# stdstu12/YUME

Hardware: AMD Instinct MI355X
Metric: denoise-steps/sec (Yume-5B 720P, 33-frame latent) (higher is better)
Workload: dtype bf16; 1 GPU; Yume-5B-720P random-init, 33-frame 704x1280 clip (latent 48x13x44x80, FramePack lfz=8, L=9460), ODE Euler steps of a 50-step shift-7 schedule, no CFG, one chain per GPU; num_layers=30, parallelism=dp1 (independent chains, replicated weights)

## Files before the change

include/yume_hip.h:

```cpp
#ifndef YUME_HIP_H
#define YUME_HIP_H

#include <stdint.h>

#ifdef __cplusplus
extern "C" {
#endif

#define YUME_OK 0
#define YUME_EINVAL (-1)
#define YUME_ELAUNCH (-2)
#define YUME_EUNSUP (-3)

const char* yume_last_error(void);
#define YUME_ABI_VERSION 9
int yume_abi_version(void);
const char* yume_target_arch(void);

int64_t yume_counter_workspace_bytes(void);
int yume_counter_workspace_init(void* ptr, int64_t bytes, void* stream);

int yume_calibrate_mfma(int64_t iters, int64_t workgroups, void* ticks, void* sink, void* stream);

int yume_adaln_modulate(const float* x, int64_t ldx, int64_t T, int64_t C, float eps,
                        const float* mul, const float* add, int64_t tab_stride,
                        const int32_t* row_idx, int add_one,
                        void* out, int64_t ldo, int out_kind, void* stream);

enum {
    YUME_EPI_BF16 = 0,
    YUME_EPI_BF16_GELU = 1,
    YUME_EPI_F32 = 2,
    YUME_EPI_RESID = 3,
    YUME_EPI_BF16_SPLITT = 4,
    YUME_EPI_BF16_GELU_ERF = 5,
    YUME_EPI_BF16_GEGLU = 6,
    YUME_EPI_MX_GELU = 7
};
int yume_gemm_bf16(const void* A, int64_t lda, const void* W, int64_t ldw, const float* bias,
                   int64_t M, int64_t N, int64_t K, int epi,
                   void* out, int64_t ldo,
                   const float* gate, int64_t gate_stride, const int32_t* row_idx,
                   void* outT, int64_t ldt, int64_t n_split,
                   int variant, void* stream);

int64_t yume_gemm_workspace_bytes(void);
int yume_gemm_bf16_ws(const void* A, int64_t lda, const void* W, int64_t ldw, const float* bias,
                      int64_t M, int64_t N, int64_t K, int epi,
                      void* out, int64_t ldo,
                      const float* gate, int64_t gate_stride, const int32_t* row_idx,
                      void* outT, int64_t ldt, int64_t n_split,
                      int variant, void* workspace, int64_t workspace_bytes, void* stream);

int yume_quant_rows_e4m3(const void* x, int64_t ldx, int64_t R, int64_t K, void* q, int64_t ldq, float* scale, void* stream);
int yume_gemm_f8(const void* Aq, int64_t lda, const float* sa, const void* Wq, int64_t ldw, const float* sw,
                 const float* bias, int64_t M, int64_t N, int64_t K, int epi, void* out, int64_t ldo,
                 const float* gate, int64_t gate_stride, const int32_t* row_idx, void* stream);
int yume_gemm_f8_splitt(const void* Aq, int64_t lda, const float* sa, const void* Wq, int64_t ldw, const float* sw,
                        const float* bias, int64_t M, int64_t N, int64_t K,
                        void* out, int64_t ldo, void* outT, int64_t ldt, int64_t n_split, void* stream);

int yume_adaln_modulate_e4m3(const float* x, int64_t ldx, int64_t T, int64_t C, float eps, const float* mul,
                             const float* add, int64_t tab_stride, const int32_t* row_idx, int add_one,
                             void* q, int64_t ldq, float* scale, void* stream);
int yume_gemm_f8_mxout(const void* Aq, int64_t lda, const float* sa, const void* Wq, int64_t ldw, const float* sw,
                       const float* bias, int64_t M, int64_t N, int64_t K, int epi, void* out, int64_t ldo,
                       void* eo, int64_t ldeo, void* stream);
int yume_gemm_f8_mx(const void* Aq, int64_t lda, const void* ea, int64_t ldea, const void* Wq, int64_t ldw, const float* sw,
                    const float* bias, int64_t M, int64_t N, int64_t K, int epi, void* out, int64_t ldo,
                    const float* gate, int64_t gate_stride, const int32_t* row_idx, void* stream);

int yume_rmsnorm_rope(void* buf, int64_t ld, int64_t T, int64_t C, int nparts,
                      const float* w, float eps, const float* rope, int64_t D, void* stream);
int yume_rmsnorm_rows_periodic(void* buf, int64_t ld, int64_t T, int64_t C, const float* w, int64_t wperiod, float eps,
                               void* stream);

#define YUME_ATTN_Q_PRESCALED 0x100
#define YUME_ATTN_KV_PADDED 0x200
int yume_attn_fwd(const void* Q, int64_t ldq, const void* K, int64_t ldk, const void* Vt, int64_t ldvt,
                  void* O, int64_t ldo, int64_t Lq, int64_t Lk, int64_t H, float scale,
                  int accumulate, int variant, void* stream);
int64_t yume_attn_workspace_bytes(int64_t Lq, int64_t Lk, int64_t H);
int yume_attn_fwd_ws(const void* Q, int64_t ldq, const void* K, int64_t ldk, const void* Vt, int64_t ldvt,
                     void* O, int64_t ldo, int64_t Lq, int64_t Lk, int64_t H, float scale,
                     int accumulate, int variant, void* workspace, int64_t workspace_bytes, void* stream);
int yume_attn_fwd_kw(const void* Q, int64_t ldq, const void* K, int64_t ldk, const void* Vt, int64_t ldvt,
                     void* O, int64_t ldo, int64_t Lq, int64_t Lk, int64_t H, float scale,
                     int accumulate, int variant, void* workspace, int64_t workspace_bytes, float last_key_weight, void* stream);
int yume_attn_fwd_seg(const void* Q, int64_t ldq, const void* const* K, int64_t ldk, const void* const* Vt, int64_t ldvt,
                      void* O, int64_t ldo, int64_t nseg, int64_t Lq_seg, int64_t seg_pitch, const int64_t* Lk, int64_t H,
                      float scale, int accumulate, int variant, const float* last_key_weight, void* stream);
int64_t yume_attn_batch_workspace_bytes(int64_t nseg, int64_t Lq_seg, int64_t Lk_seg, int64_t H);
int yume_attn_fwd_batch(const void* Q, int64_t ldq, const void* K, int64_t ldk, const void* Vt, int64_t ldvt,
                        void* O, int64_t ldo, int64_t nseg, int64_t Lq_seg, int64_t q_pitch,
                        int64_t Lk_seg, int64_t k_pitch, int64_t H, float scale, int accumulate, int variant,
                        void* workspace, int64_t workspace_bytes, void* stream);

int yume_quant_rows_mx_e4m3(const void* x, int64_t ldx, int64_t R, int64_t K, void* q, int64_t ldq, void* e, int64_t lde, void* stream);
int yume_attn_vt_mx_e4m3(const void* Vt, int64_t ldvt, int64_t C, int64_t Lk, void* Vt8, int64_t ldvt8, void* Ev, int64_t ldev, void* stream);
int yume_attn_fwd_f8mx(const void* Q8, int64_t ldq, const void* Eq, int64_t ldeq, const void* K8, int64_t ldk, const void* Ek, int64_t ldek,
                       const void* Vt8, int64_t ldvt8, const void* Ev, int64_t ldev, void* O, int64_t ldo,
                       int64_t Lq, int64_t Lk, int64_t H, void* stream);

int yume_linear_smallm_f32(const float* in, int64_t R, int64_t K, const void* W, int w_bf16,
                           const float* bias, int64_t N, int in_act, int out_act,
                           const float* add_table, float* out, void* stream);

int yume_sinusoidal_embed(const double* t, const int32_t* t_index, int64_t R, int64_t dim,
                          float* out, void* stream);

int yume_modulation_table(const float* tab, const float* e0, int64_t B, int64_t R, int64_t W,
                          float* out, void* stream);

int yume_patch_gather(const void* x, int in_bf16, int64_t Cin, int64_t F, int64_t H, int64_t W,
                      int64_t f0, int64_t nf, int64_t kh, int64_t kw,
                      void* out, int64_t Kp, void* stream);

int yume_unpatchify(const float* in, int64_t ldi, int64_t Fr, int64_t Hp, int64_t Wp,
                    int64_t ph, int64_t pw, int64_t Cout, float* out, void* stream);

int yume_cast_bf16(const float* in, int64_t ldi, int64_t rows_valid, int64_t rows, int64_t cols,
                   void* out, int64_t ldo, void* stream);
int yume_transpose_bf16(const void* in, int in_bf16, int64_t ldi, int64_t rows, int64_t cols,
                        void* out, int64_t ldo, void* stream);


enum { YUME_CONV_EPI_ADD = 16, YUME_CONV_EPI_TSPLIT = 17, YUME_CONV_EPI_RMS_SILU = 18 };
int yume_conv3d_cl(const void* x, const void* cache, int64_t ldc, int64_t Tin, int64_t Hin, int64_t Win, int64_t Cin,
                   const void* W, int64_t ldw, const float* bias, int64_t Cout,
                   int kt, int kh, int kw, int st, int sh, int sw, int pt, int ph, int pw, int ups,
                   int64_t To, int64_t Ho, int64_t Wo, int epi, void* out, int64_t ldo,
                   const void* add, int64_t ldadd, const void* zero_page, void* stream);

int yume_vae_rmsnorm_silu(const void* x, int64_t ldx, int64_t M, int64_t C, const float* gamma, const float* beta,
                          int silu, void* y, int64_t ldy, void* stream);
// ... 45 lines not shown
```

yume_amd/_lib.py:

```python
import ctypes
import os
from ctypes import c_void_p, c_int, c_int64, c_float, c_char_p

_HERE = os.path.dirname(os.path.abspath(__file__))
LIB_PATH = os.environ.get("YUME_HIP_LIB") or os.path.join(_HERE, "lib", "libyume_hip.so")

_P, _I, _L, _F = c_void_p, c_int, c_int64, c_float

SIGNATURES = {
    "yume_last_error": [],
    "yume_abi_version": [],
    "yume_target_arch": [],
    "yume_counter_workspace_bytes": [],
    "yume_counter_workspace_init": [_P, _L, _P],
    "yume_calibrate_mfma": [_L, _L, _P, _P, _P],
    "yume_adaln_modulate": [_P, _L, _L, _L, _F, _P, _P, _L, _P, _I, _P, _L, _I, _P],
    "yume_adaln_modulate_e4m3": [_P, _L, _L, _L, _F, _P, _P, _L, _P, _I, _P, _L, _P, _P],
    "yume_gemm_bf16": [_P, _L, _P, _L, _P, _L, _L, _L, _I, _P, _L, _P, _L, _P, _P, _L, _L, _I, _P],
    "yume_gemm_workspace_bytes": [],
    "yume_gemm_bf16_ws": [_P, _L, _P, _L, _P, _L, _L, _L, _I, _P, _L, _P, _L, _P, _P, _L, _L, _I, _P, _L, _P],
    "yume_quant_rows_e4m3": [_P, _L, _L, _L, _P, _L, _P, _P],
    "yume_gemm_f8": [_P, _L, _P, _P, _L, _P, _P, _L, _L, _L, _I, _P, _L, _P, _L, _P, _P],
    "yume_gemm_f8_splitt": [_P, _L, _P, _P, _L, _P, _P, _L, _L, _L, _P, _L, _P, _L, _L, _P],
    "yume_gemm_f8_mxout": [_P, _L, _P, _P, _L, _P, _P, _L, _L, _L, _I, _P, _L, _P, _L, _P],
    "yume_gemm_f8_mx": [_P, _L, _P, _L, _P, _L, _P, _P, _L, _L, _L, _I, _P, _L, _P, _L, _P, _P],
    "yume_rmsnorm_f32": [_P, _L, _L, _L, _F, _P, _P, _L, _P],
    "yume_gemm_bf16_batched": [_P, _L, _L, _P, _L, _L, _L, _L, _L, _I, _P, _L, _L, _L, _I, _P],
    "yume_gemm_splitk_workspace_bytes": [_L, _L, _I],
    "yume_gemm_bf16_splitk": [_P, _L, _P, _L, _P, _L, _L, _L, _I, _P, _L, _I, _P, _P],
    "yume_softmax_bias_rows": [_P, _L, _L, _L, _L, _P, _L, _P, _L, _L, _P],
    "yume_rmsnorm_rows_periodic": [_P, _L, _L, _L, _P, _L, _F, _P],
    "yume_rmsnorm_rope": [_P, _L, _L, _L, _I, _P, _F, _P, _L, _P],
    "yume_attn_fwd": [_P, _L, _P, _L, _P, _L, _P, _L, _L, _L, _L, _F, _I, _I, _P],
    "yume_attn_workspace_bytes": [_L, _L, _L],
    "yume_attn_fwd_ws": [_P, _L, _P, _L, _P, _L, _P, _L, _L, _L, _L, _F, _I, _I, _P, _L, _P],
    "yume_attn_fwd_kw": [_P, _L, _P, _L, _P, _L, _P, _L, _L, _L, _L, _F, _I, _I, _P, _L, _F, _P],
    "yume_attn_fwd_seg": [_P, _L, _P, _L, _P, _L, _P, _L, _L, _L, _L, _P, _L, _F, _I, _I, _P, _P],
    "yume_attn_batch_workspace_bytes": [_L, _L, _L, _L],
    "yume_attn_fwd_batch": [_P, _L, _P, _L, _P, _L, _P, _L, _L, _L, _L, _L, _L, _L, _F, _I, _I, _P, _L, _P],
    "yume_quant_rows_mx_e4m3": [_P, _L, _L, _L, _P, _L, _P, _L, _P],
    "yume_attn_vt_mx_e4m3": [_P, _L, _L, _L, _P, _L, _P, _L, _P],
    "yume_attn_fwd_f8mx": [_P, _L, _P, _L, _P, _L, _P, _L, _P, _L, _P, _L, _P, _L, _L, _L, _L, _P],
    "yume_linear_smallm_f32": [_P, _L, _L, _P, _I, _P, _L, _I, _I, _P, _P, _P],
    "yume_sinusoidal_embed": [_P, _P, _L, _L, _P, _P],
    "yume_modulation_table": [_P, _P, _L, _L, _L, _P, _P],
    "yume_patch_gather": [_P, _I, _L, _L, _L, _L, _L, _L, _L, _L, _P, _L, _P],
    "yume_unpatchify": [_P, _L, _L, _L, _L, _L, _L, _L, _P, _P],
    "yume_cast_bf16": [_P, _L, _L, _L, _L, _P, _L, _P],
    "yume_transpose_bf16": [_P, _I, _L, _L, _L, _P, _L, _P],
    "yume_conv3d_cl": [_P, _P, _L, _L, _L, _L, _L, _P, _L, _P, _L, _I, _I, _I, _I, _I, _I, _I, _I, _I, _I, _L, _L, _L, _I, _P, _L,
                       _P, _L, _P, _P],
    "yume_vae_rmsnorm_silu": [_P, _L, _L, _L, _P, _P, _I, _P, _L, _P],
    "yume_vae_rmsnorm_silu_mx": [_P, _L, _L, _L, _P, _P, _I, _P, _L, _P, _L, _P],
    "yume_conv3d_cl_f8mx": [_P, _P, _P, _P, _L, _L, _L, _L, _L, _L, _P, _L, _P, _P, _L, _I, _I, _I, _I, _I, _I, _I, _I, _I, _I, _L, _L, _L,
                            _I, _P, _L, _P, _L, _P, _P],
    "yume_conv_up2_fold": [_P, _L, _L, _L, _L, _L, _P, _L, _P, _L, _P, _L, _P],
    "yume_vae_dupup_add": [_P, _L, _L, _L, _L, _L, _P, _L, _L, _L, _I, _I, _I, _P],
    "yume_vae_avgdown_add": [_P, _L, _L, _L, _L, _L, _P, _L, _L, _I, _I, _P],
    "yume_softmax_rows": [_P, _L, _L, _L, _F, _P, _L, _P],
    "yume_vae_pack_input": [_P, _I, _L, _L, _L, _L, _I, _P, _P, _P, _L, _P],
    "yume_frames_u8": [_P, _L, _L, _L, _L, _P, _P],
    "yume_frames_u8_trunc": [_P, _L, _L, _L, _L, _P, _P],
    "yume_vae_unpack_output": [_P, _L, _L, _L, _L, _L, _I, _P, _P, _F, _F, _P, _P],
}
_RES = {"yume_last_error": c_char_p, "yume_target_arch": c_char_p, "yume_gemm_splitk_workspace_bytes": c_int64, "yume_attn_workspace_bytes": c_int64,
        "yume_attn_batch_workspace_bytes": c_int64,
        "yume_counter_workspace_bytes": c_int64, "yume_gemm_workspace_bytes": c_int64}

_lib = None
ABI_VERSION = 9


def load():
    global _lib
    if _lib is not None:
        return _lib
    if not os.path.exists(LIB_PATH):
        raise RuntimeError(
            f"{LIB_PATH} is missing: the HIP extension has not been built. "
            "Run `python -c 'import __graft_entry__ as g; g.build()'` (or `python -m yume_amd.build`). "
            "There is no CPU/PyTorch fallback for the yume_amd hot path.")
    import torch
    lib = ctypes.CDLL(LIB_PATH)
    for name, argtypes in SIGNATURES.items():
        fn = getattr(lib, name)
        fn.argtypes = argtypes
        fn.restype = _RES.get(name, c_int)
    got, arch = int(lib.yume_abi_version()), lib.yume_target_arch()
    if got != ABI_VERSION or arch != b"gfx950":
        raise RuntimeError(f"{LIB_PATH} has ABI version {got} for {arch!r}, this binding needs {ABI_VERSION} for gfx950: "
                           "rebuild with `python -m yume_amd.build --force`")
    _lib = lib
    return lib


def check(rc, what):
    if rc != 0:
        msg = load().yume_last_error()
        raise RuntimeError(f"{what} failed (rc={rc}): {msg.decode() if msg else '?'}")
```

yume_amd/csrc/gemm_bf16.hip:

```cpp
#include "gemm_core.hpp"
#include "gemm_w4.hpp"

using namespace gemm_core;

namespace {
bool w4_auto() {
    static const bool on = [] { const char* v = getenv("YUME_GEMM_W4"); return !v || atoi(v) != 0; }();
    return on;
}
bool gemm_log() {
    static const bool on = [] { const char* v = getenv("YUME_GEMM_LOG"); return v && atoi(v) != 0; }();
    return on;
}
void gemm_log_line(const char* kernel, int64_t M, int64_t N, int64_t K, int epi, int variant, int64_t lda, int64_t ldw, int64_t ldo, int64_t ldt,
                   int64_t n_split, bool ws, int64_t batch) {
    fprintf(stderr, "[gemm_bf16] %s M=%lld N=%lld K=%lld epi=%d variant=%d lda=%lld ldw=%lld ldo=%lld ldt=%lld n_split=%lld ws=%d batch=%lld\n", kernel,
            (long long)M, (long long)N, (long long)K, epi, variant, (long long)lda, (long long)ldw, (long long)ldo, (long long)ldt, (long long)n_split,
            ws ? 1 : 0, (long long)batch);
}
}

extern "C" int64_t yume_gemm_workspace_bytes(void) { return gemm_w4::sk_workspace_bytes(gemm_w4::SK_MAX_SLOTS); }

extern "C" int yume_gemm_bf16(const void* A, int64_t lda, const void* W, int64_t ldw, const float* bias, int64_t M,
                              int64_t N, int64_t K, int epi, void* out, int64_t ldo, const float* gate,
                              int64_t gate_stride, const int32_t* row_idx, void* outT, int64_t ldt, int64_t n_split,
                              int variant, void* stream) {
    return yume_gemm_bf16_ws(A, lda, W, ldw, bias, M, N, K, epi, out, ldo, gate, gate_stride, row_idx, outT, ldt, n_split, variant, nullptr, 0, stream);
}

extern "C" int yume_gemm_bf16_ws(const void* A, int64_t lda, const void* W, int64_t ldw, const float* bias, int64_t M,
                                 int64_t N, int64_t K, int epi, void* out, int64_t ldo, const float* gate,
                                 int64_t gate_stride, const int32_t* row_idx, void* outT, int64_t ldt, int64_t n_split,
                                 int variant, void* workspace, int64_t workspace_bytes, void* stream) {
    YUME_REQUIRE(A && W && out, "gemm_bf16: NULL pointer");
    YUME_REQUIRE(M > 0 && N > 0 && K > 0, "gemm_bf16: empty problem M=%lld N=%lld K=%lld", (long long)M, (long long)N, (long long)K);
    YUME_REQUIRE(M < (1ll << 31) && N < (1ll << 31) && K < (1ll << 31), "gemm_bf16: dimension too large");
    YUME_REQUIRE((K % BK) == 0, "gemm_bf16: K=%lld must be a multiple of %d", (long long)K, BK);
    YUME_REQUIRE((N % 4) == 0, "gemm_bf16: N=%lld must be a multiple of 4", (long long)N);
    YUME_REQUIRE((lda % 8) == 0 && (ldw % 8) == 0, "gemm_bf16: lda/ldw must be multiples of 8 (16-byte rows)");
    YUME_REQUIRE((ldo % 4) == 0, "gemm_bf16: ldo must be a multiple of 4");
    YUME_REQUIRE(((uintptr_t)A % 16) == 0 && ((uintptr_t)W % 16) == 0 && ((uintptr_t)out % 16) == 0, "gemm_bf16: pointers must be 16-byte aligned");
    Problem p;
    p.W = (const unsigned short*)W; p.ldw = ldw;
    p.M = (int)M; p.N = (int)N; p.K = (int)K;
    p.tiles_m = (int)((M + BM - 1) / BM);
    p.tiles_n = (int)((N + BN - 1) / BN);
    p.group_m = 8;
    p.bsW = 0; p.bsO = 0;
    bool sk = false;
    if (variant == 0 && workspace != nullptr && w4_auto() && epi != YUME_EPI_BF16_GEGLU &&
        use_256(p, 0, epi != YUME_EPI_BF16_SPLITT || (n_split % 256) == 0) && gemm_w4::w4_applies(p, lda, epi) &&
        (epi != YUME_EPI_BF16_SPLITT || (ldt % 8) == 0)) {
        Problem q = p;
        q.tiles_m = (int)((M + 255) / 256);
        q.tiles_n = (int)((N + 255) / 256);
        gemm_w4::w4_sk_plan(q, workspace, workspace_bytes);
        sk = q.sk_wgs != 0;
    }
    if (!sk && variant == 0 && epi != YUME_EPI_BF16_GEGLU && use_256(p, 0, epi != YUME_EPI_BF16_SPLITT || (n_split % 256) == 0)) {
        const int64_t tn = (N + 255) / 256, tm = (M + 255) / 256, T = tm * tn, R = T % 256, full = T - R;
        const int64_t m_main = full / tn, M_main = m_main * 256, rem = M - M_main;
        if (R > 0 && R <= 96 && full >= 256 && m_main >= 1 && rem > 0 && rem <= 1024) {
            const int64_t osz = (epi == YUME_EPI_F32 || epi == YUME_EPI_RESID) ? 4 : 2;
            auto remainder = [&](void* s2) {
                return yume_gemm_bf16(reinterpret_cast<const unsigned short*>(A) + M_main * lda, lda, W, ldw, bias, rem, N, K, epi,
                                      reinterpret_cast<char*>(out) + M_main * ldo * osz, ldo, gate, gate_stride,
                                      row_idx ? row_idx + M_main : nullptr,
                                      outT ? reinterpret_cast<unsigned short*>(outT) + M_main : nullptr, ldt, n_split, 1, s2);
            };
            int rc = yume_gemm_bf16(A, lda, W, ldw, bias, M_main, N, K, epi, out, ldo, gate, gate_stride, row_idx, outT, ldt, n_split,
                                    w4_auto() ? 3 : 2, stream);
            if (rc != YUME_OK) return rc;
            return remainder(stream);
        }
    }
    PlainA al;
    al.A = (const unsigned short*)A; al.lda = lda; al.M = (int)M; al.bsA = 0;
    Epilogue e = {};
    e.bias = bias;
    e.out = out; e.ldo = ldo;
    e.gate = gate; e.gate_stride = gate_stride; e.row_idx = row_idx;
    e.outT = (unsigned short*)outT; e.ldt = ldt; e.n_split = (int)n_split;
    hipStream_t st = (hipStream_t)stream;
    const bool split_ok = epi != YUME_EPI_BF16_SPLITT || (n_split % 256) == 0;
    const bool big = use_256(p, variant == 3 ? 2 : variant, split_ok);
    const bool w4 = (variant == 3 || (variant == 0 && big && w4_auto())) && split_ok && gemm_w4::w4_applies(p, lda, epi) &&
                    (epi != YUME_EPI_BF16_SPLITT || (ldt % 8) == 0);
    if (gemm_log())
        gemm_log_line(epi == YUME_EPI_BF16_GEGLU ? "g256" : w4 ? (sk ? "w4+sk" : "w4") : big ? "g256" : "g128", M, N, K, epi, variant, lda, ldw, ldo, ldt,
                      n_split, workspace != nullptr, 1);
#define YUME_GO(E) (w4 ? gemm_w4::launch_w4(E, p, al, e, st, "gemm_bf16", variant == 0 ? workspace : nullptr, workspace_bytes) : big ? launch256<E>(p, al, e, st, "gemm_bf16") : launch<E>(p, al, e, st, "gemm_bf16"))
    switch (epi) {
        case YUME_EPI_BF16: return YUME_GO(YUME_EPI_BF16);
        case YUME_EPI_BF16_GELU: return YUME_GO(YUME_EPI_BF16_GELU);
        case YUME_EPI_BF16_GELU_ERF: return YUME_GO(YUME_EPI_BF16_GELU_ERF);
        case YUME_EPI_F32: return YUME_GO(YUME_EPI_F32);
        case YUME_EPI_RESID:
            YUME_REQUIRE(gate == nullptr || (gate_stride % 4) == 0, "gemm_bf16: gate_stride must be a multiple of 4");
            return YUME_GO(YUME_EPI_RESID);
        case YUME_EPI_BF16_GEGLU:
            YUME_REQUIRE((N % 8) == 0 && bias == nullptr, "gemm_bf16: GEGLU needs N %% 8 == 0 and no bias");
            return launch256<YUME_EPI_BF16_GEGLU>(p, al, e, st, "gemm_bf16");
        case YUME_EPI_BF16_SPLITT:
            YUME_REQUIRE(outT != nullptr && n_split >= 0 && (n_split % BN) == 0 && ldt >= M && (ldt % 4) == 0,
                         "gemm_bf16: SPLITT needs outT, n_split %% 128 == 0, ldt >= M and ldt %% 4 == 0");
            YUME_REQUIRE(((uintptr_t)outT % 16) == 0, "gemm_bf16: outT must be 16-byte aligned");
            return YUME_GO(YUME_EPI_BF16_SPLITT);
        default:
            yume_set_error("gemm_bf16: unknown epilogue %d", epi);
            return YUME_EINVAL;
    }
}

extern "C" int yume_gemm_bf16_batched(const void* A, int64_t lda, int64_t strideA, const void* W, int64_t ldw, int64_t strideW,
                                      int64_t M, int64_t N, int64_t K, int epi, void* out, int64_t ldo, int64_t strideO,
                                      int64_t batch, int variant, void* stream) {
    (void)variant;
    YUME_REQUIRE(A && W && out, "gemm_bf16_batched: NULL pointer");
    YUME_REQUIRE(epi == YUME_EPI_BF16 || epi == YUME_EPI_F32, "gemm_bf16_batched: only the plain bf16 / fp32 epilogues");
    YUME_REQUIRE(batch >= 1 && batch <= 65535, "gemm_bf16_batched: batch %lld", (long long)batch);
    YUME_REQUIRE(M > 0 && N > 0 && K > 0 && M < (1ll << 31) && N < (1ll << 31) && K < (1ll << 31), "gemm_bf16_batched: bad problem size");
    YUME_REQUIRE((K % BK) == 0 && (N % 4) == 0, "gemm_bf16_batched: K must be a multiple of %d and N of 4", BK);
    YUME_REQUIRE((lda % 8) == 0 && (ldw % 8) == 0 && (ldo % 4) == 0, "gemm_bf16_batched: lda/ldw must be multiples of 8, ldo of 4");
    YUME_REQUIRE((strideA % 8) == 0 && (strideW % 8) == 0 && (strideO % 8) == 0, "gemm_bf16_batched: strides must keep 16-byte alignment");
    YUME_REQUIRE(((uintptr_t)A % 16) == 0 && ((uintptr_t)W % 16) == 0 && ((uintptr_t)out % 16) == 0, "gemm_bf16_batched: pointers must be 16-byte aligned");
    Problem p;
    p.W = (const unsigned short*)W; p.ldw = ldw;
    p.M = (int)M; p.N = (int)N; p.K = (int)K;
    p.tiles_m = (int)((M + BM - 1) / BM);
    p.tiles_n = (int)((N + BN - 1) / BN);
    p.group_m = 8;
    p.bsW = strideW;
    p.bsO = strideO * (epi == YUME_EPI_F32 ? 4 : 2);
    PlainA al;
    al.A = (const unsigned short*)A; al.lda = lda; al.M = (int)M; al.bsA = strideA;
    Epilogue e = {};
    e.out = out; e.ldo = ldo;
    hipStream_t st = (hipStream_t)stream;
    if (gemm_log()) gemm_log_line("batched", M, N, K, epi, variant, lda, ldw, ldo, 0, 0, false, batch);
    if (epi == YUME_EPI_F32) return launch<YUME_EPI_F32>(p, al, e, st, "gemm_bf16_batched", (int)batch);
    return launch<YUME_EPI_BF16>(p, al, e, st, "gemm_bf16_batched", (int)batch);
}

namespace {
template <int EPI>
__global__ __launch_bounds__(256) void splitk_reduce_kernel(const float* __restrict__ ws, int splits, int64_t MN, int N,
                                                            const float* __restrict__ bias, void* __restrict__ out, int64_t ldo) {
    const int64_t nq = MN >> 2;
    for (int64_t i = (int64_t)blockIdx.x * blockDim.x + threadIdx.x; i < nq; i += (int64_t)gridDim.x * blockDim.x) {
        f32x4 v = *reinterpret_cast<const f32x4*>(ws + 4 * i);
        for (int s = 1; s < splits; ++s) v += *reinterpret_cast<const f32x4*>(ws + s * MN + 4 * i);
        const int64_t m = (4 * i) / N;
        const int n = (int)((4 * i) - m * N);
        if (bias) v += *reinterpret_cast<const f32x4*>(bias + n);
        if (EPI == YUME_EPI_F32) {
            *reinterpret_cast<f32x4*>(reinterpret_cast<float*>(out) + m * ldo + n) = v;
        } else if (EPI == YUME_EPI_RESID) {
            float* xo = reinterpret_cast<float*>(out) + m * ldo + n;
            *reinterpret_cast<f32x4*>(xo) = *reinterpret_cast<const f32x4*>(xo) + v;
        } else if (EPI == YUME_EPI_BF16_GEGLU) {
            const unsigned o = pack_bf16x2(v[1] * gelu_tanh(v[0]), v[3] * gelu_tanh(v[2]));
            *reinterpret_cast<unsigned*>(reinterpret_cast<unsigned short*>(out) + m * ldo + (n >> 1)) = o;
        } else {
            if (EPI == YUME_EPI_BF16_GELU) {
#pragma unroll
                for (int q = 0; q < 4; ++q) v[q] = gelu_tanh(v[q]);
// ... 50 lines not shown
```

yume_amd/csrc/gemm_w4.hpp:

```cpp
#pragma once
#include "gemm_core.hpp"
#include "trace.hpp"

namespace gemm_w4 {
using namespace gemm_core;

constexpr int NTHR_W4 = 256;
constexpr int OPER_BYTES = 256 * 128;
constexpr int BUF_BYTES = 2 * OPER_BYTES;
constexpr int LDS_W4 = 2 * BUF_BYTES;

#define W4_AG8(n) "a" #n "0", "a" #n "1", "a" #n "2", "a" #n "3", "a" #n "4", "a" #n "5", "a" #n "6", "a" #n "7", "a" #n "8", "a" #n "9"
#define W4_AGPRS "a0", "a1", "a2", "a3", "a4", "a5", "a6", "a7", "a8", "a9", W4_AG8(1), W4_AG8(2), W4_AG8(3), W4_AG8(4), W4_AG8(5), W4_AG8(6), \
    W4_AG8(7), W4_AG8(8), W4_AG8(9), W4_AG8(10), W4_AG8(11), W4_AG8(12), W4_AG8(13), W4_AG8(14), W4_AG8(15), W4_AG8(16), W4_AG8(17), W4_AG8(18), \
    W4_AG8(19), W4_AG8(20), W4_AG8(21), W4_AG8(22), W4_AG8(23), W4_AG8(24), "a250", "a251", "a252", "a253", "a254", "a255"

#define W4_MFMA2(T0, X0, Y0, T1, X1, Y1)                                                                                                         \
    asm volatile("v_mfma_f32_16x16x32_bf16 a[%c4:%c5], %0, %1, a[%c4:%c5]\n\tv_mfma_f32_16x16x32_bf16 a[%c6:%c7], %2, %3, a[%c6:%c7]"             \
                 ::"v"(X0), "v"(Y0), "v"(X1), "v"(Y1), "n"((T0) * 4), "n"((T0) * 4 + 3), "n"((T1) * 4), "n"((T1) * 4 + 3) : "memory", W4_AGPRS)
#define W4_MFMA2_DMA(T0, X0, Y0, T1, X1, Y1, voff, sbase, lbase, loff)                                                                            \
    asm volatile("s_add_u32 m0, %10, %11\n\tv_mfma_f32_16x16x32_bf16 a[%c4:%c5], %0, %1, a[%c4:%c5]\n\tglobal_load_lds_dwordx4 %8, %9\n\t"         \
                 "v_mfma_f32_16x16x32_bf16 a[%c6:%c7], %2, %3, a[%c6:%c7]"                                                                       \
                 ::"v"(X0), "v"(Y0), "v"(X1), "v"(Y1), "n"((T0) * 4), "n"((T0) * 4 + 3), "n"((T1) * 4), "n"((T1) * 4 + 3), "v"(voff), "s"(sbase),   \
                 "s"(lbase), "n"(loff) : "memory", "scc", W4_AGPRS)
// ... 550 lines not shown
            tails = true;
            const int ntail = (p.sk_s - 1) * R;
            pc0 = (w - R) * p.sk_q;
            pc1 = min(ntail, pc0 + p.sk_q);
            if (pc0 >= pc1) return;
        }
    }
    for (int pc = pc0; pc < pc1; ++pc) {
        int t = head_t, j = 0, k0 = 0, k1 = nk, slot = -1, nslice = 1;
        if (p.sk_wgs && (int)blockIdx.x >= ndp) {
            if (tails) {
                j = 1 + pc / R;
                t = pc - (j - 1) * R;
                k0 = p.sk_lh + (j - 1) * p.sk_lt;
                k1 = j == p.sk_s - 1 ? nk : k0 + p.sk_lt;
                slot = pc;
            } else {
                k1 = p.sk_lh;
                nslice = p.sk_s;
            }
        }
        int m0, n0;
        tile_origin(p, tile0 + t, m0, n0);
        if (epi == YUME_EPI_BF16_SPLITT && n0 >= e.n_split) {
            w4_mainloop<false>(p, al, smem, m0, n0, k0, k1 - k0);
            w4_finish_piece<false>(p, e, epi, smem, m0, n0, slot, t, nslice);
        } else {
            w4_mainloop<true>(p, al, smem, m0, n0, k0, k1 - k0);
            w4_finish_piece<true>(p, e, epi, smem, m0, n0, slot, t, nslice);
        }
        if (pc + 1 < pc1) __syncthreads();
    }
    TRACE_STAMP(2);
}

inline bool w4_applies(const Problem& p, int64_t lda, int epi) {
    if (p.K < 3 * BK) return false;
#ifdef W4_EXPERIMENT
    if (epi != YUME_EPI_BF16) return false;
#endif
    if (255ll * lda * 2 + 128 >= (1ll << 32) || 255ll * p.ldw * 2 + 128 >= (1ll << 32)) return false;
    return epi == YUME_EPI_BF16 || epi == YUME_EPI_BF16_GELU || epi == YUME_EPI_BF16_GELU_ERF || epi == YUME_EPI_F32 || epi == YUME_EPI_RESID ||
           epi == YUME_EPI_BF16_SPLITT;
}

inline void w4_sk_plan(Problem& p, void* ws, int64_t ws_bytes) {
    p.sk_dp = 0; p.sk_tiles = 0; p.sk_wgs = 0; p.sk_s = 1; p.sk_q = 1; p.sk_lh = 0; p.sk_lt = 0; p.sk_ws = nullptr;
    static const bool on = [] { const char* v = getenv("YUME_GEMM_SK"); return !v || atoi(v) != 0; }();
    static const int ncu = [] {
        int d = 0, n = 0;
        if (hipGetDevice(&d) != hipSuccess || hipDeviceGetAttribute(&n, hipDeviceAttributeMultiprocessorCount, d) != hipSuccess) n = 0;
        return n;
    }();
    if (!on || ws == nullptr || ncu < 64 || ncu > SK_MAX_SLOTS || (ncu & 7) != 0) return;
    if (ws_bytes < sk_workspace_bytes(SK_MAX_SLOTS) || ((uintptr_t)ws & 15) != 0) return;
    const int T = p.tiles_m * p.tiles_n, nk = p.K / BK;
    const int R = T % ncu;
    if (R == 0 || T < ncu) return;
    static const int min_nk = [] { const char* v = getenv("YUME_GEMM_SK_MIN_NK"); return v ? atoi(v) : 96; }();
    if (nk < min_nk) return;
    int s, q, lh, lt;
    if (2 * R > ncu) {
        s = 2;
        q = (R + (ncu - R) - 1) / (ncu - R);
        lt = nk / (q + 1);
        lh = nk - lt;
    } else {
        s = ncu / R;
        if (s > nk / SK_MIN_KT) s = nk / SK_MIN_KT;
        q = 1;
        lt = nk / s;
        lh = lt;
    }
    if (s < 2 || lt < SK_MIN_KT || lh < SK_MIN_KT || (s - 1) * R > SK_MAX_SLOTS) return;
    const int nwg = R + ((s - 1) * R + q - 1) / q;
    if (nwg > ncu) return;
    p.sk_tiles = R;
    p.sk_dp = T - R;
    p.sk_s = s; p.sk_q = q; p.sk_lh = lh; p.sk_lt = lt;
    p.sk_wgs = (nwg + 7) / 8 * 8;
    p.sk_ws = (char*)ws;
}

inline int launch_w4(int epi, const Problem& p128, const PlainA& al, const Epilogue& e, hipStream_t st, const char* what, void* ws = nullptr,
                     int64_t ws_bytes = 0) {
    Problem p = p128;
    p.tiles_m = (p.M + 255) / 256;
    p.tiles_n = (p.N + 255) / 256;
    p.group_m = g_group_m;
    { static const int d = [] { const char* v = getenv("YUME_GEMM_EPI_DIRECT"); return v ? atoi(v) : 0; }(); p.epi_direct = d; }
    w4_sk_plan(p, ws, ws_bytes);
    const unsigned grid = p.sk_wgs ? (unsigned)(p.sk_dp + p.sk_wgs) : (unsigned)(p.tiles_m * p.tiles_n);
    hipLaunchKernelGGL(gemm_w4_kernel<0>, dim3(grid), dim3(NTHR_W4), 0, st, p, al, e, epi);
    YUME_CHECK_LAUNCH(what);
    return YUME_OK;
}

}
```

Baseline: 10.04 denoise-steps/sec.

## Split tail-wave GEMM rows into a narrow-N band kernel to fill the last wave

Adds a planner that, when the 256x256 tile count leaves a partial last wave over the CUs, splits the GEMM into a main part of full waves and a leftover row band. The band runs in a new 256x192-tile kernel variant so it has more, smaller tiles and keeps more CUs busy. The band kernel has its own MFMA/DMA schedule and BF16/RESID epilogues. It is on by default but costs an extra launch and adds a large hand-scheduled kernel that could hide correctness problems.

```diff
diff --git a/include/yume_hip.h b/include/yume_hip.h
--- a/include/yume_hip.h
+++ b/include/yume_hip.h
@@ -51,6 +51,8 @@
                       const float* gate, int64_t gate_stride, const int32_t* row_idx,
                       void* outT, int64_t ldt, int64_t n_split,
                       int variant, void* workspace, int64_t workspace_bytes, void* stream);
+
+int yume_gemm_band(int on);
 
 int yume_quant_rows_e4m3(const void* x, int64_t ldx, int64_t R, int64_t K, void* q, int64_t ldq, float* scale, void* stream);
 int yume_gemm_f8(const void* Aq, int64_t lda, const float* sa, const void* Wq, int64_t ldw, const float* sw,
diff --git a/yume_amd/_lib.py b/yume_amd/_lib.py
--- a/yume_amd/_lib.py
+++ b/yume_amd/_lib.py
@@ -18,6 +18,7 @@
     "yume_adaln_modulate_e4m3": [_P, _L, _L, _L, _F, _P, _P, _L, _P, _I, _P, _L, _P, _P],
     "yume_gemm_bf16": [_P, _L, _P, _L, _P, _L, _L, _L, _I, _P, _L, _P, _L, _P, _P, _L, _L, _I, _P],
     "yume_gemm_workspace_bytes": [],
+    "yume_gemm_band": [_I],
     "yume_gemm_bf16_ws": [_P, _L, _P, _L, _P, _L, _L, _L, _I, _P, _L, _P, _L, _P, _P, _L, _L, _I, _P, _L, _P],
     "yume_quant_rows_e4m3": [_P, _L, _L, _L, _P, _L, _P, _P],
     "yume_gemm_f8": [_P, _L, _P, _P, _L, _P, _P, _L, _L, _L, _I, _P, _L, _P, _L, _P, _P],
diff --git a/yume_amd/csrc/gemm_band_plan.hpp b/yume_amd/csrc/gemm_band_plan.hpp
--- /dev/null
+++ b/yume_amd/csrc/gemm_band_plan.hpp
@@ -0,0 +1,39 @@
+#pragma once
+#include <stdint.h>
+
+namespace gemm_band {
+
+constexpr int BAND_N = 192;
+constexpr int BAND_M = 256;
+constexpr int BAND_COST_NUM = 3;
+constexpr int BAND_COST_DEN = 4;
+constexpr int BAND_MIN_CUS = 64;
+constexpr int BAND_MAX_CUS = 256;
+
+struct Plan {
+    int take;
+    int64_t m_main;
+    int64_t band_rows;
+    int64_t band_tiles;
+};
+
+static inline Plan plan(int64_t M, int64_t N, int ncu) {
+    Plan p = {0, 0, 0, 0};
+    if (ncu < BAND_MIN_CUS || ncu > BAND_MAX_CUS || (ncu & 7) != 0) return p;
+    if (M <= 0 || N <= 0 || (N % BAND_N) != 0) return p;
+    const int64_t tm = (M + 255) / 256, tn = (N + 255) / 256, T = tm * tn;
+    const int64_t full = (T / ncu) * ncu;
+    const int64_t m_main = full / tn;
+    if (m_main < 1 || m_main >= tm) return p;
+    const int64_t band_rows = tm - m_main, band_tiles = band_rows * (N / BAND_N);
+    if (band_tiles > ncu) return p;
+    const int64_t rounds_main = (m_main * tn + ncu - 1) / ncu, rounds_all = (T + ncu - 1) / ncu;
+    if (BAND_COST_DEN * rounds_main + BAND_COST_NUM >= BAND_COST_DEN * rounds_all) return p;
+    p.take = 1;
+    p.m_main = m_main;
+    p.band_rows = band_rows;
+    p.band_tiles = band_tiles;
+    return p;
+}
+
+}
diff --git a/yume_amd/csrc/gemm_bf16.hip b/yume_amd/csrc/gemm_bf16.hip
--- a/yume_amd/csrc/gemm_bf16.hip
+++ b/yume_amd/csrc/gemm_bf16.hip
@@ -1,9 +1,26 @@
 #include "gemm_core.hpp"
 #include "gemm_w4.hpp"
+#include "gemm_band_plan.hpp"
 
 using namespace gemm_core;
 
+namespace gemm_w4 {
+int launch_w4_band(int epi, const Problem& p128, const PlainA& al, const Epilogue& e, hipStream_t st, const char* what);
+}
+
 namespace {
+int& band_flag() {
+    static int on = [] { const char* v = getenv("YUME_GEMM_BAND"); return (!v || atoi(v) != 0) ? 1 : 0; }();
+    return on;
+}
+int device_cus() {
+    static const int ncu = [] {
+        int d = 0, n = 0;
+        if (hipGetDevice(&d) != hipSuccess || hipDeviceGetAttribute(&n, hipDeviceAttributeMultiprocessorCount, d) != hipSuccess) n = 0;
+        return n;
+    }();
+    return ncu;
+}
 bool w4_auto() {
     static const bool on = [] { const char* v = getenv("YUME_GEMM_W4"); return !v || atoi(v) != 0; }();
     return on;
@@ -21,6 +38,13 @@
 }
 
 extern "C" int64_t yume_gemm_workspace_bytes(void) { return gemm_w4::sk_workspace_bytes(gemm_w4::SK_MAX_SLOTS); }
+
+extern "C" int yume_gemm_band(int on) {
+    int& f = band_flag();
+    const int prev = f;
+    f = on ? 1 : 0;
+    return prev;
+}
 
 extern "C" int yume_gemm_bf16(const void* A, int64_t lda, const void* W, int64_t ldw, const float* bias, int64_t M,
                               int64_t N, int64_t K, int epi, void* out, int64_t ldo, const float* gate,
@@ -75,6 +99,18 @@
             return remainder(stream);
         }
     }
+    if (!sk && variant == 0 && band_flag() && (epi == YUME_EPI_BF16 || epi == YUME_EPI_RESID) && w4_auto() && use_256(p, 0, true) &&
+        gemm_w4::w4_applies(p, lda, epi)) {
+        const gemm_band::Plan bp = gemm_band::plan(M, N, device_cus());
+        if (bp.take) {
+            const int64_t M_main = bp.m_main * 256, osz = epi == YUME_EPI_RESID ? 4 : 2;
+            int rc = yume_gemm_bf16(A, lda, W, ldw, bias, M_main, N, K, epi, out, ldo, gate, gate_stride, row_idx, outT, ldt, n_split, 3, stream);
+            if (rc != YUME_OK) return rc;
+            return yume_gemm_bf16(reinterpret_cast<const unsigned short*>(A) + M_main * lda, lda, W, ldw, bias, M - M_main, N, K, epi,
+                                  reinterpret_cast<char*>(out) + M_main * ldo * osz, ldo, gate, gate_stride, row_idx ? row_idx + M_main : nullptr,
+                                  outT, ldt, n_split, 4, stream);
+        }
+    }
     PlainA al;
     al.A = (const unsigned short*)A; al.lda = lda; al.M = (int)M; al.bsA = 0;
     Epilogue e = {};
@@ -83,6 +119,14 @@
     e.gate = gate; e.gate_stride = gate_stride; e.row_idx = row_idx;
     e.outT = (unsigned short*)outT; e.ldt = ldt; e.n_split = (int)n_split;
     hipStream_t st = (hipStream_t)stream;
+    if (variant == 4) {
+        YUME_REQUIRE((N % gemm_band::BAND_N) == 0, "gemm_bf16: variant 4 needs N %% %d == 0 (N=%lld)", gemm_band::BAND_N, (long long)N);
+        YUME_REQUIRE(epi == YUME_EPI_BF16 || epi == YUME_EPI_RESID, "gemm_bf16: variant 4 takes the BF16 and RESID epilogues only (epi=%d)", epi);
+        YUME_REQUIRE(gemm_w4::w4_applies(p, lda, epi), "gemm_bf16: variant 4 needs K >= %d and 32-bit row offsets inside a tile", 3 * BK);
+        YUME_REQUIRE(epi != YUME_EPI_RESID || gate == nullptr || (gate_stride % 4) == 0, "gemm_bf16: gate_stride must be a multiple of 4");
+        if (gemm_log()) gemm_log_line("w4b", M, N, K, epi, variant, lda, ldw, ldo, ldt, n_split, false, 1);
+        return gemm_w4::launch_w4_band(epi, p, al, e, st, "gemm_bf16");
+    }
     const bool split_ok = epi != YUME_EPI_BF16_SPLITT || (n_split % 256) == 0;
     const bool big = use_256(p, variant == 3 ? 2 : variant, split_ok);
     const bool w4 = (variant == 3 || (variant == 0 && big && w4_auto())) && split_ok && gemm_w4::w4_applies(p, lda, epi) &&
diff --git a/yume_amd/csrc/gemm_w4.hpp b/yume_amd/csrc/gemm_w4.hpp
--- a/yume_amd/csrc/gemm_w4.hpp
+++ b/yume_amd/csrc/gemm_w4.hpp
@@ -656,6 +656,7 @@
     p.sk_ws = (char*)ws;
 }
 
+#ifndef GEMM_W4_NO_LAUNCH
 inline int launch_w4(int epi, const Problem& p128, const PlainA& al, const Epilogue& e, hipStream_t st, const char* what, void* ws = nullptr,
                      int64_t ws_bytes = 0) {
     Problem p = p128;
@@ -669,5 +670,6 @@
     YUME_CHECK_LAUNCH(what);
     return YUME_OK;
 }
-
-}
+#endif
+
+}
diff --git a/yume_amd/csrc/gemm_w4_band.hip b/yume_amd/csrc/gemm_w4_band.hip
--- /dev/null
+++ b/yume_amd/csrc/gemm_w4_band.hip
@@ -0,0 +1,18 @@
+#define GEMM_W4_NO_LAUNCH
+#include "gemm_w4_band.hpp"
+
+namespace gemm_w4 {
+
+int launch_w4_band(int epi, const Problem& p128, const PlainA& al, const Epilogue& e, hipStream_t st, const char* what) {
+    Problem p = p128;
+    p.tiles_m = (p.M + 255) / 256;
+    p.tiles_n = p.N / WB_N;
+    p.group_m = g_group_m;
+    { static const int d = [] { const char* v = getenv("YUME_GEMM_EPI_DIRECT"); return v ? atoi(v) : 0; }(); p.epi_direct = d; }
+    p.sk_dp = 0; p.sk_tiles = 0; p.sk_wgs = 0; p.sk_s = 1; p.sk_q = 1; p.sk_lh = 0; p.sk_lt = 0; p.sk_ws = nullptr;
+    hipLaunchKernelGGL(gemm_w4_band_kernel<0>, dim3((unsigned)(p.tiles_m * p.tiles_n)), dim3(NTHR_W4), 0, st, p, al, e, epi);
+    YUME_CHECK_LAUNCH(what);
+    return YUME_OK;
+}
+
+}
diff --git a/yume_amd/csrc/gemm_w4_band.hpp b/yume_amd/csrc/gemm_w4_band.hpp
--- /dev/null
+++ b/yume_amd/csrc/gemm_w4_band.hpp
@@ -0,0 +1,292 @@
+#pragma once
+#include "gemm_w4.hpp"
+#include "gemm_band_plan.hpp"
+
+namespace gemm_w4 {
+
+constexpr int WB_N = gemm_band::BAND_N;
+constexpr int WB_SLOTS = 48;
+constexpr int WB_PIECES = 14;
+constexpr int WB_FRAGS = 14;
+constexpr int WB_BAR_A = 15;
+constexpr int WB_BAR_B = 30;
+constexpr int WB_DMA0 = WB_BAR_A + 2;
+constexpr int WB_F0_FIRST = WB_BAR_B + 2;
+constexpr int wb_dma_pos(int q) { return WB_DMA0 + (q * (WB_SLOTS - 1 - WB_DMA0)) / (WB_PIECES - 1); }
+constexpr int wb_piece_at(int pos) {
+    for (int q = 0; q < WB_PIECES; ++q)
+        if (wb_dma_pos(q) == pos) return q;
+    return -1;
+}
+constexpr int wb_pieces_before_bar_b() {
+    int k = 0;
+    for (int q = 0; q < WB_PIECES; ++q) k += wb_dma_pos(q) <= WB_BAR_B ? 1 : 0;
+    return k;
+}
+constexpr bool wb_positions_distinct() {
+    for (int q = 1; q < WB_PIECES; ++q)
+        if (wb_dma_pos(q) <= wb_dma_pos(q - 1)) return false;
+    return true;
+}
+static_assert(WB_F0_FIRST + WB_FRAGS <= WB_SLOTS && wb_dma_pos(WB_PIECES - 1) <= WB_SLOTS - 1 && WB_FRAGS - 1 < WB_BAR_A &&
+              wb_dma_pos(0) > WB_BAR_A && wb_positions_distinct(), "the plan must fit the 48 slots");
+constexpr int wb_wpiece(int q) { return (q - 8) + ((q - 8) >= 3 ? 1 : 0); }
+constexpr int wb_piece_loff(int q) { return q < 8 ? q * 4096 : OPER_BYTES + wb_wpiece(q) * 4096; }
+
+#define WB_T(g) ((((g) % 48) / 6) * 8 + ((g) % 6))
+#define WB_X(g) c.fb[(g) / 48][(g) % 6]
+#define WB_Y(g) c.fa[(g) / 48][((g) % 48) / 6]
+
+template <int g, bool DMA>
+__device__ __forceinline__ void wb_gaps(Ctx& c) {
+    if constexpr (g < 2 * WB_SLOTS) {
+        constexpr int pos = g >> 1;
+        constexpr int q = DMA ? wb_piece_at(pos) : -1;
+        if constexpr (q >= 0 && q < 8)
+            W4_MFMA2_DMA(WB_T(g), WB_X(g), WB_Y(g), WB_T(g + 1), WB_X(g + 1), WB_Y(g + 1), c.va[q & 7], c.pa, c.lcur, wb_piece_loff(q & 15));
+        else if constexpr (q >= 8)
+            W4_MFMA2_DMA(WB_T(g), WB_X(g), WB_Y(g), WB_T(g + 1), WB_X(g + 1), WB_Y(g + 1), c.vb[wb_wpiece(q & 15) & 7], c.pb, c.lcur, wb_piece_loff(q & 15));
+        else
+            W4_MFMA2(WB_T(g), WB_X(g), WB_Y(g), WB_T(g + 1), WB_X(g + 1), WB_Y(g + 1));
+        if constexpr (pos < WB_FRAGS) {
+            if constexpr (pos < 6) c.fb[1][pos % 6] = w4_frag(c, c.rb1 + (pos % 6) * 2048);
+            else c.fa[1][(pos - 6) & 7] = w4_frag(c, c.ra1 + ((pos - 6) & 7) * 2048);
+        }
+        if constexpr (pos == WB_BAR_A) asm volatile("s_waitcnt lgkmcnt(0)\n\ts_barrier" ::: "memory");
+        if constexpr (pos == WB_BAR_B) {
+            constexpr int keep = DMA ? wb_pieces_before_bar_b() : 0;
+            asm volatile("s_waitcnt vmcnt(%c0)\n\ts_barrier" ::"n"(keep) : "memory");
+        }
+        if constexpr (pos >= WB_F0_FIRST && pos < WB_F0_FIRST + WB_FRAGS) {
+            constexpr int r = pos - WB_F0_FIRST;
+            if constexpr (r < 6) c.fb[0][r % 6] = w4_frag(c, c.rb0n + (r % 6) * 2048);
+            else c.fa[0][(r - 6) & 7] = w4_frag(c, c.ra0n + ((r - 6) & 7) * 2048);
+        }
+        wb_gaps<g + 2, DMA>(c);
+    }
+}
+template <int q>
+__device__ __forceinline__ void wb_stage_all(Ctx& c) {
+    if constexpr (q < WB_PIECES) {
+        if constexpr (q < 8) W4_DMA(c.va[q & 7], c.pa, c.lcur, wb_piece_loff(q));
+        else W4_DMA(c.vb[wb_wpiece(q) & 7], c.pb, c.lcur, wb_piece_loff(q));
+        wb_stage_all<q + 1>(c);
+    }
+}
+
+template <bool DMA>
+__device__ __forceinline__ void wb_loop(Ctx& c, int t0, int t1, unsigned lbase) {
+    for (int t = t0; t < t1; ++t) {
+        wb_gaps<0, DMA>(c);
+        if constexpr (DMA) {
+            c.pa += 128;
+            c.pb += 128;
+        }
+        c.lcur = lbase + (((t + 1) & 1) ? BUF_BYTES : 0);
+        c.ra1 ^= BUF_BYTES;
+        c.rb1 ^= BUF_BYTES;
+        c.ra0n ^= BUF_BYTES;
+        c.rb0n ^= BUF_BYTES;
+    }
+}
+
+__device__ __forceinline__ void wb_mainloop(const Problem& p, const PlainA& al, char* smem, int m0, int n0, int nk) {
+    const int tid = threadIdx.x;
+    const int lane = tid & 63;
+    const int wave = __builtin_amdgcn_readfirstlane(tid >> 6);
+    const int wr = wave >> 1, wc = wave & 1;
+    Ctx c;
+    c.smem = smem;
+    const unsigned lbase = (unsigned)(uintptr_t)(__attribute__((address_space(3))) char*)smem + wave * 1024;
+    c.lcur = lbase;
+    c.pa = reinterpret_cast<const char*>(al.A + (int64_t)m0 * al.lda);
+    c.pb = reinterpret_cast<const char*>(p.W + (int64_t)n0 * p.ldw);
+    const unsigned lda_b = (unsigned)al.lda * 2u, ldw_b = (unsigned)p.ldw * 2u;
+    {
+        const int rl = 8 * wave + (lane >> 3);
+        const unsigned ch = (unsigned)(((lane & 7) ^ (rl & 7)) << 4);
+        const int mleft = p.M - 1 - m0, nleft = p.N - 1 - n0;
+#pragma unroll
+        for (int j = 0; j < 8; ++j) {
+            c.va[j] = (unsigned)min(32 * j + rl, mleft) * lda_b + ch;
+            c.vb[j] = (unsigned)min((j >> 2) * 96 + (j & 3) * 32 + rl, nleft) * ldw_b + ch;
+        }
+    }
+    const unsigned sw0 = (unsigned)(((lane >> 4) ^ (lane & 7)) << 4), sw1 = (unsigned)(((4 | (lane >> 4)) ^ (lane & 7)) << 4);
+    const unsigned rowa = wr * 16384 + (lane & 15) * 128, rowb = OPER_BYTES + wc * 16384 + (lane & 15) * 128;
+    wb_stage_all<0>(c);
+    c.pa += 128;
+    c.pb += 128;
+    c.lcur = lbase + BUF_BYTES;
+    wb_stage_all<0>(c);
+    c.pa += 128;
+    c.pb += 128;
+    c.lcur = lbase;
+    acc_zero<0, 256>();
+    asm volatile("s_waitcnt vmcnt(%c0)\n\ts_barrier" ::"n"(WB_PIECES) : "memory");
+#pragma unroll
+    for (int r = 0; r < 6; ++r) c.fb[0][r] = w4_frag(c, rowb + sw0 + r * 2048);
+#pragma unroll
+    for (int r = 0; r < 8; ++r) c.fa[0][r] = w4_frag(c, rowa + sw0 + r * 2048);
+    c.ra1 = rowa + sw1;
+    c.rb1 = rowb + sw1;
+    c.ra0n = BUF_BYTES + rowa + sw0;
+    c.rb0n = BUF_BYTES + rowb + sw0;
+    wb_loop<true>(c, 0, nk - 2, lbase);
+    wb_loop<false>(c, nk - 2, nk, lbase);
+    asm volatile("s_waitcnt lgkmcnt(0)\n\ts_barrier" ::: "memory");
+    asm volatile("s_nop 15\n\ts_nop 15" ::: "memory");
+}
+
+__device__ __forceinline__ void wb_store_image(char* smem, unsigned short* dst, int64_t ld, int row0, int rows_valid, int col0) {
+    const int lane = threadIdx.x & 63;
+    const int wave = __builtin_amdgcn_readfirstlane(threadIdx.x >> 6);
+    const int l31 = lane & 31, rh = lane >> 5;
+    const bool act = l31 < WB_N / 8;
+    const unsigned lrow = (unsigned)((wave * 64 + rh) * 512), lch = (unsigned)((l31 ^ rh) << 4);
+    char* o = reinterpret_cast<char*>(dst + col0 + l31 * 8) + (int64_t)(row0 + wave * 64 + rh) * ld * 2;
+    const int64_t step = ld * 4;
+    const int rleft = act ? rows_valid - wave * 64 - rh : 0;
+#pragma unroll
+    for (int g = 0; g < 4; ++g) {
+        u32x4 d[8];
+#pragma unroll
+        for (int u = 0; u < 8; ++u) {
+            const int it = g * 8 + u;
+            d[u] = *reinterpret_cast<const u32x4*>(smem + lrow + it * 1024 + (lch ^ (unsigned)(32 * (it & 15))));
+        }
+#pragma unroll
+        for (int u = 0; u < 8; ++u) {
+            const int it = g * 8 + u;
+            if (2 * it < rleft) *reinterpret_cast<u32x4*>(o + it * step) = d[u];
+        }
+    }
+}
+
+template <int EPI>
+__device__ __forceinline__ void wb_epilogue(const Problem& p, const Epilogue& e, int m0, int n0, char* smem) {
+    static_assert(EPI == YUME_EPI_BF16 || EPI == YUME_EPI_RESID, "the band kernel takes the plain bf16 and the residual epilogue");
+    const int lane = threadIdx.x & 63;
+    const int wave = __builtin_amdgcn_readfirstlane(threadIdx.x >> 6);
+    const int wr = wave >> 1, wc = wave & 1;
+    const int l15 = lane & 15, l4 = lane >> 4;
+    if constexpr (EPI == YUME_EPI_BF16) {
+        if (!p.epi_direct && (e.ldo % 8) == 0) {
+            f32x4 b[6];
+#pragma unroll
+            for (int j = 0; j < 6; ++j)
+                b[j] = e.bias ? *reinterpret_cast<const f32x4*>(e.bias + n0 + wc * 96 + 16 * j + 4 * l4) : f32x4{0.f, 0.f, 0.f, 0.f};
+            unsigned oe[6], oo[6];
+            const unsigned base = (unsigned)((wr * 128 + l15) * 512 + (l4 & 1) * 8);
+#pragma unroll
+            for (int j = 0; j < 6; ++j) {
+                const unsigned cj = (unsigned)(12 * wc + 2 * j + (l4 >> 1));
+                oe[j] = base + ((cj ^ (unsigned)l15) << 4);
+                oo[j] = base + ((cj ^ (unsigned)(16 + l15)) << 4);
+            }
+            asm volatile("s_waitcnt lgkmcnt(0)\n\ts_barrier" ::: "memory");
+            static_for<0, 8>([&](auto ii) {
+                constexpr int i = decltype(ii)::value;
+                static_for<0, 6>([&](auto jj) {
+                    constexpr int j = decltype(jj)::value;
+                    const f32x4 v = acc_tile<i * 8 + j>() + b[j];
+                    u32x2 o;
+                    o[0] = pack_bf16x2(v[0], v[1]);
+                    o[1] = pack_bf16x2(v[2], v[3]);
+                    *reinterpret_cast<u32x2*>(smem + ((i & 1) ? oo[j] : oe[j]) + i * 8192) = o;
+                });
+            });
+            asm volatile("s_waitcnt lgkmcnt(0)\n\ts_barrier" ::: "memory");
+            wb_store_image(smem, reinterpret_cast<unsigned short*>(e.out), e.ldo, m0, min(256, p.M - m0), n0);
+            return;
+        }
+    }
+    if constexpr (EPI == YUME_EPI_RESID) {
+        f32x4 b[6];
+#pragma unroll
+        for (int j = 0; j < 6; ++j)
+            b[j] = e.bias ? *reinterpret_cast<const f32x4*>(e.bias + n0 + wc * 96 + 16 * j + 4 * l4) : f32x4{0.f, 0.f, 0.f, 0.f};
+        const int mrow = m0 + wr * 128 + l15, ncol = n0 + wc * 96 + 4 * l4;
+        const bool ragged_m = m0 + 256 > p.M;
+        const int mlast = p.M - 1 - mrow;
+        float* const xo = reinterpret_cast<float*>(e.out) + (int64_t)mrow * e.ldo + ncol;
+        const int64_t xstep = 16 * e.ldo;
+        auto xoff = [&](int i) -> int64_t { return ragged_m ? (int64_t)(min(16 * i, mlast)) * e.ldo : i * xstep; };
+        const bool gated = e.gate != nullptr;
+        bool rowed = gated && e.row_idx != nullptr;
+        int ridx[8];
+#pragma unroll
+        for (int i = 0; i < 8; ++i) ridx[i] = rowed ? e.row_idx[min(mrow + 16 * i, p.M - 1)] : 0;
+        f32x4 x[2][6], g[2][6];
+        auto issue_x = [&](auto ii, auto bb) {
+            constexpr int i = decltype(ii)::value, bf = decltype(bb)::value;
+#pragma unroll
+            for (int j = 0; j < 6; ++j) x[bf][j] = *reinterpret_cast<const f32x4*>(xo + xoff(i) + 16 * j);
+        };
+        auto issue_g = [&](auto ii, auto bb) {
+            constexpr int i = decltype(ii)::value, bf = decltype(bb)::value;
+            if (rowed || (gated && i < 2)) {
+                const float* gp = e.gate + (int64_t)ridx[i] * e.gate_stride + ncol;
+#pragma unroll
+                for (int j = 0; j < 6; ++j) g[bf][j] = *reinterpret_cast<const f32x4*>(gp + 16 * j);
+            }
+        };
+        issue_x(std::integral_constant<int, 0>{}, std::integral_constant<int, 0>{});
+        issue_x(std::integral_constant<int, 1>{}, std::integral_constant<int, 1>{});
+        if (rowed) {
+            const int r0 = __builtin_amdgcn_readfirstlane(ridx[0]);
+            bool same = true;
+#pragma unroll
+            for (int i = 0; i < 8; ++i) same &= ridx[i] == r0;
+            if (__all(same)) rowed = false;
+        }
+        issue_g(std::integral_constant<int, 0>{}, std::integral_constant<int, 0>{});
+        issue_g(std::integral_constant<int, 1>{}, std::integral_constant<int, 1>{});
+        static_for<0, 8>([&](auto ii) {
+            constexpr int i = decltype(ii)::value, bf = i & 1;
+            static_for<0, 6>([&](auto jj) {
+                constexpr int j = decltype(jj)::value;
+                const f32x4 v = acc_tile<i * 8 + j>() + b[j];
+                if (gated) x[bf][j] += v * g[bf][j];
+                else x[bf][j] += v;
+                if (!ragged_m || 16 * i <= mlast) *reinterpret_cast<f32x4*>(xo + i * xstep + 16 * j) = x[bf][j];
+            });
+            if constexpr (i + 2 < 8) {
+                issue_x(std::integral_constant<int, i + 2>{}, std::integral_constant<int, bf>{});
+                issue_g(std::integral_constant<int, i + 2>{}, std::integral_constant<int, bf>{});
+            }
+        });
+        return;
+    }
+    static_for<0, 8>([&](auto ii) {
+        constexpr int i = decltype(ii)::value;
+        static_for<0, 6>([&](auto jj) {
+            constexpr int j = decltype(jj)::value;
+            const f32x4 v = acc_tile<i * 8 + j>();
+            const int m = m0 + wr * 128 + 16 * i + l15, n = n0 + wc * 96 + 16 * j + 4 * l4;
+            if (m < p.M && n < p.N) store_row4<EPI>(v, m, n, p, e);
+        });
+    });
+}
+
+__device__ __forceinline__ void wb_origin(const Problem& p, int wg, int& m0, int& n0) {
+    const int width = p.group_m * p.tiles_n;
+    const int group = wg / width;
+    const int first_m = group * p.group_m;
+    const int gsz = min(p.tiles_m - first_m, p.group_m);
+    m0 = (first_m + (wg % width) % gsz) * 256;
+    n0 = ((wg % width) / gsz) * WB_N;
+}
+
+template <int UNUSED = 0>
+__global__ __launch_bounds__(NTHR_W4, 1) void gemm_w4_band_kernel(Problem p, PlainA al, Epilogue e, int epi) {
+    __shared__ __attribute__((aligned(16))) char smem[LDS_W4];
+    int start, count, m0, n0;
+    xcd_chunk(p.tiles_m * p.tiles_n, blockIdx.x & 7, start, count);
+    wb_origin(p, start + (blockIdx.x >> 3), m0, n0);
+    wb_mainloop(p, al, smem, m0, n0, p.K / BK);
+    if (epi == YUME_EPI_RESID) wb_epilogue<YUME_EPI_RESID>(p, e, m0, n0, smem);
+    else wb_epilogue<YUME_EPI_BF16>(p, e, m0, n0, smem);
+}
+
+}
```

Result: no change. 10.08 denoise-steps/sec (median of 6 runs) (+0.4%).
